# EvolBioInf/andi

Hardware: AMD Instinct MI355X
Metric: genome-pairs/sec (ordered pairs, n^2-n) over the N x N anchor-distance loop (higher is better)
Workload: dtype u8

## Files before the change

andi_amd/csrc/api.hip:

```cpp
#include <hip/hip_runtime.h>

#include <algorithm>
#include <atomic>
#include <chrono>
#include <cstdarg>
#include <cstdio>
#include <cstdlib>
#include <cstring>
#include <mutex>
#include <string>
#include <thread>
#include <sys/mman.h>
#include <vector>

#include "api_internal.h"
#include "andi_dev.h"
#include "andi_hip.h"
#include "bootstrap.h"
#include "dev_arena.h"
#include "esa_build.h"
#include "knobs.h"
#include "sa_device.h"
#include "scan.h"

// ... 620 lines not shown
	return 0;
}

int andi_hip_esa_build_index(andi_hip_ctx *ctx, andi_hip_esa *e) {
	if (!ctx || !e) return 1;
	HIP_TRY(ctx, hipSetDevice(ctx->device));
	Timed t(ctx, 0);
	const int ext = andi_index_single_ext(ctx->queries_hint, e->rec_valid);
	hipError_t err = andi_launch_index_build(build_args(e), ext, ctx->stream);
	t.stop();
	if (err == hipSuccess) err = hipEventRecord(ctx->built, ctx->stream);
	if (err != hipSuccess) return fail(ctx, "andi_hip_esa_build_index", err);
	e->index_built = true, e->deep_ext = (ext == 2 && !e->rec_valid) ? 0 : ext, ctx->builds_pending = true;
	return 0;
}

int andi_hip_esa_build_index_batch(andi_hip_ctx *ctx, andi_hip_esa *const *esas, size_t count) {
	if (!ctx || !esas || count == 0 || count > 65535) {
		if (ctx) ctx->err = "andi_hip_esa_build_index_batch: bad arguments";
		return 1;
	}
	HIP_TRY(ctx, hipSetDevice(ctx->device));
	if (ctx->ib_cap < count) {
		HIP_TRY(ctx, hipStreamSynchronize(ctx->stream));
		if (ctx->ib_dev) (void)andi_arena::dev_free(ctx->ib_dev);
		if (ctx->ib_host) host_pool::pinned_put(ctx->ib_host, ctx->ib_cap * sizeof(AndiIndexBatchItem));
		ctx->ib_dev = ctx->ib_host = nullptr, ctx->ib_cap = 0;
		const size_t cap = std::max<size_t>(count, 64);
		HIP_TRY(ctx, andi_arena::dev_malloc(&ctx->ib_dev, cap * sizeof(AndiIndexBatchItem)));
		HIP_TRY(ctx, host_pool::pinned_get(&ctx->ib_host, cap * sizeof(AndiIndexBatchItem)));
		if (!ctx->ib_done) HIP_TRY(ctx, hipEventCreateWithFlags(&ctx->ib_done, hipEventDisableTiming));
		ctx->ib_cap = cap;
	} else {
		HIP_TRY(ctx, hipEventSynchronize(ctx->ib_done));
	}
	auto *items = (AndiIndexBatchItem *)ctx->ib_host;
	int32_t max_n = 0;
	for (size_t k = 0; k < count; ++k) {
		andi_hip_esa *e = esas[k];
		if (!e) {
			ctx->err = "andi_hip_esa_build_index_batch: null subject";
			return 1;
		}
		items[k].S = e->S, items[k].SA = e->SA, items[k].deep = e->deep, items[k].N0 = e->N0, items[k].N1 = e->N1, items[k].P = e->P;
		items[k].flags = e->flags, items[k].n = e->n, items[k].deepK = e->deepK;
		items[k].rec = e->rec_valid ? e->rec : nullptr;
		items[k].rec2 = e->rec_valid ? e->rec2 : nullptr;
		items[k].single_ext = andi_index_single_ext(ctx->queries_hint, e->rec_valid);
		max_n = std::max(max_n, e->n);
	}
	Timed t(ctx, 0);
	hipError_t err = hipMemcpyAsync(ctx->ib_dev, ctx->ib_host, count * sizeof(AndiIndexBatchItem), hipMemcpyHostToDevice, ctx->stream);
	if (err == hipSuccess) err = hipEventRecord(ctx->ib_done, ctx->stream);
	if (err == hipSuccess) err = andi_launch_index_build_batch((const AndiIndexBatchItem *)ctx->ib_dev, (uint32_t)count, max_n, ctx->stream);
	t.stop();
	if (err == hipSuccess) err = hipEventRecord(ctx->built, ctx->stream);
	if (err != hipSuccess) return fail(ctx, "andi_hip_esa_build_index_batch", err);
	for (size_t k = 0; k < count; ++k) {
		const int ext = items[k].single_ext;
		esas[k]->index_built = true, esas[k]->deep_ext = (ext == 2 && !esas[k]->rec_valid) ? 0 : ext;
	}
	ctx->builds_pending = true;
	return 0;
}

int andi_hip_esa_flags(andi_hip_ctx *ctx, const andi_hip_esa *e, int32_t *out4) {
	if (!ctx || !e || !out4) return 1;
	HIP_TRY(ctx, hipStreamSynchronize(ctx->stream));
	memcpy(out4, e->h_flags, 4 * sizeof(int32_t));
	return 0;
}

int andi_hip_esa_download(andi_hip_ctx *ctx, const andi_hip_esa *e, int32_t *LCP, int32_t *CLD,
						  uint8_t *FVC, andi_hip_interval *cache) {
	if (!ctx || !e) return 1;
	if (!e->ref_built) {
		ctx->err = "andi_hip_esa_download: reference arrays not built (call andi_hip_esa_build)";
		return 1;
	}
	const size_t n = (size_t)e->n;
	HIP_TRY(ctx, hipStreamSynchronize(ctx->stream));
	if (LCP) HIP_TRY(ctx, hipMemcpy(LCP, e->LCP, (n + 1) * 4, hipMemcpyDeviceToHost));
	if (CLD) HIP_TRY(ctx, hipMemcpy(CLD, e->CLD, (n + 1) * 4, hipMemcpyDeviceToHost));
	if (FVC) HIP_TRY(ctx, hipMemcpy(FVC, e->FVC, n, hipMemcpyDeviceToHost));
	if (cache)
		HIP_TRY(ctx, hipMemcpy(cache, e->tab, ((size_t)16 << (2 * ANDI_CACHE_K)), hipMemcpyDeviceToHost));
	return 0;
}

int andi_hip_esa_download_index(andi_hip_ctx *ctx, const andi_hip_esa *e, uint32_t *table, int *K) {
	if (!ctx || !e) return 1;
	if (!e->index_built) {
		ctx->err = "andi_hip_esa_download_index: scan index not built (call andi_hip_esa_build_index)";
		return 1;
	}
	if (K) *K = e->deepK;
	HIP_TRY(ctx, hipStreamSynchronize(ctx->stream));
	if (table) HIP_TRY(ctx, hipMemcpy(table, e->deep, (size_t)8 << (2 * e->deepK), hipMemcpyDeviceToHost));
	return 0;
}

int andi_hip_esa_single_form(const andi_hip_esa *e) { return e && e->index_built ? e->deep_ext : 0; }

void andi_hip_esa_free(andi_hip_ctx *ctx, andi_hip_esa *e) {
	if (!e) return;
	if (ctx) (void)hipSetDevice(ctx->device);
	(void)hipDeviceSynchronize();
// ... 407 lines not shown
```

andi_amd/csrc/esa_build.h:

```cpp
#pragma once
#include <hip/hip_runtime.h>
#include <stdint.h>

#define ANDI_MIN_LEVELS 6

struct MinTree {
	const int32_t *lv[ANDI_MIN_LEVELS];
	int32_t cnt[ANDI_MIN_LEVELS];
	int levels;
};

struct EsaBuildArgs {
	const uint8_t *S;
	const int32_t *SA;
	int32_t *LCP;
	int32_t *CLD;
	uint8_t *FVC;
	int4 *tab;
	uint2 *deep;
	uint8_t *N0, *N1;
	uint32_t *P;
	int32_t *flags;
	const uint32_t *rec;
	const uint16_t *rec2;
	int32_t deepK;
	int32_t *min_scratch;
	int32_t n;
};

struct AndiIndexBatchItem {
	const uint8_t *S;
	const int32_t *SA;
	uint2 *deep;
	uint8_t *N0, *N1;
	uint32_t *P;
	int32_t *flags;
	const uint32_t *rec;
	const uint16_t *rec2;
	int32_t n, deepK;
	int32_t single_ext;
};

size_t andi_min_tree_entries(int32_t n);
int andi_index_single_ext(size_t queries, bool sorted_on_device);
hipError_t andi_launch_index_build_batch(const AndiIndexBatchItem *d_items, uint32_t count, int32_t max_n, hipStream_t st);
hipError_t andi_launch_pack_symbols_batch(const AndiIndexBatchItem *d_items, uint32_t count, size_t bytes, hipStream_t st);
hipError_t andi_launch_pack_planes_batch(const AndiIndexBatchItem *d_items, uint32_t count, size_t max_n, hipStream_t st);
hipError_t andi_launch_esa_build(const EsaBuildArgs &a, hipStream_t st);
hipError_t andi_launch_index_build(const EsaBuildArgs &a, int single_ext, hipStream_t st);
hipError_t andi_launch_rs_from_query(uint8_t *RS, const uint8_t *q, uint32_t len, hipStream_t st);
hipError_t andi_launch_gc_counts(const uint8_t *pool, const uint64_t *d_off, const uint32_t *d_len, uint32_t nq, uint32_t longest,
								 unsigned long long *d_counts, hipStream_t st);
hipError_t andi_launch_sep_counts(const uint8_t *pool, const uint64_t *d_off, const uint32_t *d_len, uint32_t nq, uint32_t longest,
								  uint32_t *d_counts, hipStream_t st);
```

andi_amd/csrc/esa_build.hip:

```cpp
#include "andi_dev.h"
#include "esa_build.h"
#include "scan.h"
#include "knobs.h"

#include <cstring>

#define CHECK_LAUNCH()                                                                             \
	do {                                                                                           \
		hipError_t e_ = hipGetLastError();                                                         \
		if (e_ != hipSuccess) return e_;                                                           \
	} while (0)

__global__ __launch_bounds__(256) void k_phi_scatter(const int32_t *__restrict__ SA,
													 int32_t *__restrict__ phi, int32_t n) {
	int32_t r = blockIdx.x * blockDim.x + threadIdx.x;
	if (r >= n) return;
	int32_t prev = r ? SA[r - 1] : -1;
	phi[SA[r]] = prev;
}

#define PLCP_CHUNK 32
__global__ __launch_bounds__(256) void k_plcp_chunks(const uint8_t *__restrict__ S,
													 int32_t *__restrict__ phi_plcp, int32_t n) {
	int64_t chunk = (int64_t)blockIdx.x * blockDim.x + threadIdx.x;
// ... 197 lines not shown
	}
	auto squeeze = [](uint32_t x) {
		x &= 0x33333333u;
		x = (x | (x >> 2)) & 0x0f0f0f0fu;
		x = (x | (x >> 4)) & 0x00ff00ffu;
		x = (x | (x >> 8)) & 0x0000ffffu;
		return x;
	};
	uint32_t y = __brev(squeeze((uint32_t)w) | (squeeze((uint32_t)(w >> 32)) << 16));
	y = ((y & 0x55555555u) << 1) | ((y >> 1) & 0x55555555u);
	return ((y >> (32 - 2 * K)) << 6) | (sep << 4) | v;
}

__device__ __forceinline__ uint32_t rec_lcp(uint32_t a, uint32_t b, int K) {
	uint32_t x = REC_CODE(a) ^ REC_CODE(b);
	uint32_t same = x ? (uint32_t)(__builtin_clz(x) - (32 - 2 * K)) >> 1 : (uint32_t)K;
	uint32_t va = REC_V(a), vb = REC_V(b);
	uint32_t m = va < vb ? va : vb;
	return same < m ? same : m;
}

__device__ __forceinline__ uint32_t rec_lcp_code(uint32_t code, uint32_t a, int K) {
	uint32_t x = code ^ REC_CODE(a);
	uint32_t same = x ? (uint32_t)(__builtin_clz(x) - (32 - 2 * K)) >> 1 : (uint32_t)K;
	uint32_t va = REC_V(a);
	return same < va ? same : va;
}

#ifndef PT_BLOCK
#define PT_BLOCK 256
#endif
#ifndef PT_GAPS
#define PT_GAPS 3
#endif
#define PT_TILE (PT_BLOCK * PT_GAPS)
#define PT_WORDS (PT_TILE / 64)
#define PT_RANKED 4096
__device__ __forceinline__ uint32_t wave_scan_incl(uint32_t v) {
	v += (uint32_t)__builtin_amdgcn_update_dpp(0, (int)v, 0x111, 0xf, 0xf, false);
	v += (uint32_t)__builtin_amdgcn_update_dpp(0, (int)v, 0x112, 0xf, 0xf, false);
	v += (uint32_t)__builtin_amdgcn_update_dpp(0, (int)v, 0x114, 0xf, 0xf, false);
	v += (uint32_t)__builtin_amdgcn_update_dpp(0, (int)v, 0x118, 0xf, 0xf, false);
	v += (uint32_t)__builtin_amdgcn_update_dpp(0, (int)v, 0x142, 0xa, 0xf, false);
	v += (uint32_t)__builtin_amdgcn_update_dpp(0, (int)v, 0x143, 0xc, 0xf, false);
	return v;
}

__device__ __forceinline__ uint32_t first_code(bool has, uint32_t L, int K) {
	const uint32_t v = REC_V(L), sh = 2 * ((uint32_t)K - v);
	const uint32_t c = ((REC_CODE(L) >> sh) << sh) + (v == (uint32_t)K ? 1u : 0u);
	return has ? c : 0u;
}

__device__ __forceinline__ void probe_table_block(const uint8_t *__restrict__ N0, const int32_t *__restrict__ SA,
												  const uint32_t *__restrict__ REC, const uint16_t *__restrict__ REC2, uint2 *__restrict__ deep,
												  int32_t *__restrict__ flags, int32_t n, int K, int single_ext, uint32_t block) {
	__shared__ uint32_t s_first[PT_TILE];
	__shared__ uint32_t s_absent[PT_TILE];
	__shared__ uint32_t s_h[PT_TILE + 2];
	__shared__ uint2 s_present[PT_TILE];
	__shared__ uint32_t s_rec[PT_TILE + 5];
	__shared__ uint64_t s_some[PT_WORDS];
	__shared__ uint32_t s_bits[PT_RANKED / 32];
	__shared__ uint32_t s_before[PT_RANKED / 32];
	__shared__ uint16_t s_owner[PT_TILE];

	const uint32_t r0 = block * PT_TILE;
	const uint32_t lane = threadIdx.x & 63u, wave = threadIdx.x >> 6;
	auto make_rec = [&](int32_t j) { return REC ? REC[j] : suffix_rec(N0, SA, j, K); };
	uint32_t mine2[PT_GAPS];
	{
		uint32_t mine[PT_GAPS];
#pragma unroll
		for (int u = 0; u < PT_GAPS; ++u) {
			const uint32_t g = r0 + threadIdx.x + u * PT_BLOCK;
			mine[u] = g < (uint32_t)n ? make_rec((int32_t)g) : 0u;
			mine2[u] = (single_ext == 2 && REC2 && g < (uint32_t)n) ? REC2[g] : 0u;
		}
#pragma unroll
		for (int u = 0; u < PT_GAPS; ++u) s_rec[threadIdx.x + u * PT_BLOCK + 2] = mine[u];
	}
	if (threadIdx.x < 2) s_rec[threadIdx.x] = r0 + threadIdx.x >= 2 ? make_rec((int32_t)(r0 + threadIdx.x - 2)) : 0u;
	if (threadIdx.x == 2) s_rec[PT_TILE + 2] = r0 + PT_TILE < (uint32_t)n ? make_rec((int32_t)(r0 + PT_TILE)) : 0u;
	if (threadIdx.x < PT_RANKED / 32) s_bits[threadIdx.x] = 0;
	__syncthreads();
	auto rec = [&](int32_t j) {
		const uint32_t k = (uint32_t)j - r0 + 2;
		return k < PT_TILE + 3 ? s_rec[k] : make_rec(j);
	};
	const uint32_t full = (uint32_t)K;
	if (threadIdx.x == 0) s_h[0] = r0 >= 2 ? rec_lcp(s_rec[0], s_rec[1], K) : 0u;
	if (threadIdx.x == 1) s_h[PT_TILE + 1] = r0 + PT_TILE < (uint32_t)n ? rec_lcp(s_rec[PT_TILE + 1], s_rec[PT_TILE + 2], K) : 0u;

	uint32_t counts[PT_GAPS], firsts[PT_GAPS];
#pragma unroll
	for (int u = 0; u < PT_GAPS; ++u) {
		const uint32_t i = threadIdx.x + u * PT_BLOCK;
		const uint32_t gid = r0 + i;
		const bool live = gid <= (uint32_t)n;
		const int32_t r = (int32_t)(live ? gid : 0);
		const bool hasL = live && r > 0, hasR = live && r < n;
		const uint32_t Lr = s_rec[i + 1], Rr = s_rec[i + 2], a1 = s_rec[i + 3], a2 = s_rec[i + 4], a3 = s_rec[i + 5];
		const uint32_t L = hasL ? Lr : 0u, R = hasR ? Rr : 0u;
		const uint32_t sa_r = hasR ? (uint32_t)SA[r] : 0u;
		const uint32_t h = (hasL && hasR) ? rec_lcp(L, R, K) : 0u;
		s_h[i + 1] = h;
		uint32_t absent = 0, first = 1u << (2 * K), owns_present = 0;
		uint2 present = make_uint2(0, 0);

		if (live) {
			if (hasR && REC_V(R) == full && !(hasL && L == R)) {
				const bool in_tile = i + 5 < PT_TILE + 3;
				const int32_t m = a1 != R ? 0 : (a2 != R ? 1 : (a3 != R ? 2 : 3));
				int32_t j = in_tile ? r + m : r;
				const bool more = !in_tile || m == 3;
				if (more) {
					while (j + 1 < n && j - r < 16 && rec(j + 1) == R) ++j;
					if (j - r == 16 && j + 1 < n && rec(j + 1) == R) {
						int32_t lo = j + 1, hi = n - 1;
						while (lo < hi) {
							const int32_t mid = lo + ((hi - lo + 1) >> 1);
							if (rec(mid) == R) lo = mid; else hi = mid - 1;
						}
						j = lo;
					}
				}
				if (j == r) {
					const uint32_t pos = sa_r, e0 = pos + full;
					if (single_ext == 2 && REC2) {
						const uint32_t w = mine2[u];
						present = make_uint2(pos, DEEP_SINGLE | ((w >> 8) << 2) | ((w & 0xffu) << 6));
					} else if (single_ext != 1) {
						present = make_uint2(pos, DEEP_SINGLE | (1u << 2) | (full << 8));
					} else {
						const uint64_t w = ld_u64_unaligned((g_u8p)N0 + (e0 >> 1)) >> (4 * (e0 & 1u));
						uint32_t nval = (uint32_t)__builtin_ctzll((w & 0x4444444444444444ull) | (1ull << 52)) >> 2;
						auto squeeze = [](uint32_t x) {
							x &= 0x33333333u;
							x = (x | (x >> 2)) & 0x0f0f0f0fu;
							x = (x | (x >> 4)) & 0x00ff00ffu;
							x = (x | (x >> 8)) & 0x0000ffffu;
							return x;
						};
						const uint32_t ext = (squeeze((uint32_t)w) | (squeeze((uint32_t)(w >> 32)) << 16)) & ((1u << (2 * nval)) - 1u);
						present = make_uint2(pos, DEEP_SINGLE | (nval << 2) | (ext << 6));
					}
				} else {
					const bool fits = (uint32_t)(j - r) < (1u << 24);
					present = make_uint2(fits ? (uint32_t)r : 0u, fits ? DEEP_MULTI | ((uint32_t)(j - r) << 8) : (uint32_t)DEEP_SEARCH);
				}
				owns_present = 1;
			}

			if (__builtin_amdgcn_ballot_w64(hasR && (REC_SEP(R) == 1 || REC_SEP(R) == 2)) != 0 && hasR) {
				uint32_t k = REC_V(R), sp = REC_SEP(R);
				if (k >= 1 && k <= 8 && k < full && (sp == 1 || sp == 2) && (!hasL || h < k)) {
					int32_t j = r;
					while (j + 1 < n) {
						uint32_t X = rec(j + 1);
						if (REC_V(X) == k && REC_SEP(X) == sp && rec_lcp(R, X, K) == k) ++j; else break;
					}
					if (j > r && (j + 1 == n || rec_lcp(R, rec(j + 1), K) < k)) flags[0] = 1;
				}
			}

			const int32_t lo = (int32_t)first_code(hasL, L, K);
			const uint32_t shR = 2 * (full - REC_V(R));
			const int32_t hi = hasR ? (int32_t)((REC_CODE(R) >> shR) << shR) - 1 : (int32_t)((1u << (2 * K)) - 1u);
			if (lo <= hi) absent = (uint32_t)(hi - lo + 1);
			first = (uint32_t)lo;
		}
		s_first[i] = first, s_absent[i] = absent, s_present[i] = present;
		counts[u] = absent + owns_present, firsts[u] = first;
		const uint64_t b = __ballot(counts[u] != 0);
		if (lane == 0) s_some[u * (PT_BLOCK / 64) + wave] = b;
	}

	__syncthreads();
	const uint32_t base = first_code(r0 > 0, s_rec[1], K);
	const uint32_t total = (r0 + PT_TILE <= (uint32_t)n ? first_code(true, s_rec[PT_TILE + 1], K) : (1u << (2 * K))) - base;
	uint32_t owners_before;
	{
		const uint32_t mine = lane < PT_WORDS ? (uint32_t)__builtin_popcountll(s_some[lane]) : 0u;
		owners_before = wave_scan_incl(mine) - mine;
	}
#pragma unroll
	for (int u = 0; u < PT_GAPS; ++u) {
		const uint32_t word = u * (PT_BLOCK / 64) + wave;
		const uint32_t before = (uint32_t)__builtin_amdgcn_readlane((int)owners_before, __builtin_amdgcn_readfirstlane((int)word));
		if (counts[u] == 0) continue;
		const uint32_t i = threadIdx.x + u * PT_BLOCK, off = firsts[u] - base;
		s_owner[before + (uint32_t)__builtin_popcountll(s_some[word] & ((1ull << lane) - 1ull))] = (uint16_t)i;
		if (off < PT_RANKED) atomicOr(&s_bits[off >> 5], 1u << (off & 31u));
	}
	__syncthreads();
	if (wave == 0) {
		uint32_t carry = 0;
		for (uint32_t w0 = 0; w0 < PT_RANKED / 32; w0 += 64) {
			const uint32_t mine = (uint32_t)__builtin_popcount(s_bits[w0 + lane]), incl = wave_scan_incl(mine);
			s_before[w0 + lane] = carry + incl - mine;
			carry += (uint32_t)__builtin_amdgcn_readlane((int)incl, 63);
		}
	}
	__syncthreads();

	auto write_entry = [&](uint32_t t, uint32_t a) {
		const uint32_t c = base + t;
		const bool is_present = c - s_first[a] >= s_absent[a];
		const uint2 pres = s_present[a];
		const uint32_t rr = r0 + a;
		const bool gL = rr > 0, gR = rr < (uint32_t)n;
		const uint32_t gl = s_rec[a + 1], gr = s_rec[a + 2], hll = s_h[a], hrr = s_h[a + 2];
		const uint32_t xL = rec_lcp_code(c, gl, K), xR = rec_lcp_code(c, gr, K);
		const uint32_t lL = gL ? xL : 0u, lR = gR ? xR : 0u;
		const bool left = lL > lR, right = lR > lL;
		const uint32_t l = left ? lL : lR;
		const uint32_t idx = left ? rr - 1 : (right ? rr : 0u);
		const bool alone = left ? (rr < 2 || hll < l) : (rr + 1 >= (uint32_t)n || hrr < l);
		const uint32_t uniq = ((left || right) && l != 0) ? (alone ? 1u : 0u) : (n == 1 ? 1u : 0u);
		const uint2 val = is_present ? pres : make_uint2(idx, DEEP_FINAL | (uniq << 2) | (l << 8));
		__builtin_nontemporal_store(((unsigned long long)val.y << 32) | val.x, (unsigned long long *)(deep + c));
	};
	const uint32_t ranked = total < PT_RANKED ? total : PT_RANKED;
	for (uint32_t t = threadIdx.x; t < ranked; t += PT_BLOCK) {
		const uint32_t word = t >> 5;
		write_entry(t, s_owner[s_before[word] + (uint32_t)__builtin_popcount(s_bits[word] & (0xffffffffu >> (31u - (t & 31u)))) - 1u]);
	}
	for (uint32_t t = PT_RANKED + threadIdx.x; t < total; t += PT_BLOCK) {
		const uint32_t c = base + t;
		uint32_t a = 0, b = PT_TILE;
		while (b - a > 1) {
			const uint32_t mid = (a + b) >> 1;
			if (s_first[mid] <= c) a = mid; else b = mid;
		}
		write_entry(t, a);
	}
}

__global__ __launch_bounds__(PT_BLOCK) void k_probe_table(const uint8_t *__restrict__ N0, const int32_t *__restrict__ SA,
														  const uint32_t *__restrict__ rec, const uint16_t *__restrict__ rec2, uint2 *__restrict__ deep,
														  int32_t *__restrict__ flags, int32_t n, int K, int single_ext) {
	probe_table_block(N0, SA, rec, rec2, deep, flags, n, K, single_ext, blockIdx.x);
}

__global__ __launch_bounds__(PT_BLOCK) void k_probe_table_batch(const AndiIndexBatchItem *__restrict__ items) {
	const AndiIndexBatchItem it = items[blockIdx.y];
	if ((uint64_t)blockIdx.x * PT_TILE > (uint64_t)it.n) return;
	probe_table_block(it.N0, it.SA, it.rec, it.rec2, it.deep, it.flags, it.n, it.deepK, it.single_ext, blockIdx.x);
}

size_t andi_min_tree_entries(int32_t n) {
	size_t total = 0;
	size_t cnt = (size_t)n + 1;
	while (cnt > 64) {
		cnt = (cnt + 63) / 64;
		total += cnt;
	}
	return total ? total : 1;
}

int andi_index_single_ext(size_t queries, bool sorted_on_device) {
	const int coop = andi_coop_enabled();
	if (coop == 0) return 0;
	if (sorted_on_device) return 2;
	return (coop > 0 || queries >= 256) ? 1 : 0;
}

hipError_t andi_launch_index_build(const EsaBuildArgs &a, int single_ext, hipStream_t st) {
	const int32_t n = a.n;
	hipError_t e;
	e = andi_launch_pack_symbols(a.S, (size_t)n + 1 + 64, a.N0, a.N1, a.flags + 1, st);
	if (e != hipSuccess) return e;
	if (a.P) e = andi_launch_pack_planes(a.N0, (size_t)n + 1 + 64, a.P, st);
	if (e != hipSuccess) return e;
	k_probe_table<<<(unsigned)(((int64_t)n + 1 + PT_TILE - 1) / PT_TILE), PT_BLOCK, 0, st>>>(a.N0, a.SA, a.rec, a.rec2, a.deep, a.flags, n,
																				  a.deepK, single_ext);
	CHECK_LAUNCH();
	return hipSuccess;
}

hipError_t andi_launch_index_build_batch(const AndiIndexBatchItem *d_items, uint32_t count, int32_t max_n, hipStream_t st) {
	if (count == 0) return hipSuccess;
	hipError_t e = andi_launch_pack_symbols_batch(d_items, count, (size_t)max_n + 1 + 64, st);
	if (e != hipSuccess) return e;
	e = andi_launch_pack_planes_batch(d_items, count, (size_t)max_n, st);
	if (e != hipSuccess) return e;
	const dim3 grid((unsigned)(((int64_t)max_n + 1 + PT_TILE - 1) / PT_TILE), count);
	k_probe_table_batch<<<grid, PT_BLOCK, 0, st>>>(d_items);
	CHECK_LAUNCH();
	return hipSuccess;
}

hipError_t andi_launch_esa_build(const EsaBuildArgs &a, hipStream_t st) {
	const int32_t n = a.n;
	const int B = 256;
	auto blocks = [&](int64_t items) { return (unsigned)((items + B - 1) / B); };

	int32_t *plcp = a.CLD;
	k_phi_scatter<<<blocks(n), B, 0, st>>>(a.SA, plcp, n);
	CHECK_LAUNCH();
	int64_t chunks = ((int64_t)n + PLCP_CHUNK - 1) / PLCP_CHUNK;
	k_plcp_chunks<<<blocks(chunks), B, 0, st>>>(a.S, plcp, n);
	CHECK_LAUNCH();
	k_lcp_fvc<<<blocks((int64_t)n + 1), B, 0, st>>>(a.S, a.SA, plcp, a.LCP, a.FVC, n);
	CHECK_LAUNCH();

	MinTree t;
	t.lv[0] = a.LCP;
	t.cnt[0] = n + 1;
	t.levels = 1;
	int32_t *next = a.min_scratch;
	while (t.cnt[t.levels - 1] > 64 && t.levels < ANDI_MIN_LEVELS) {
		int32_t in_cnt = t.cnt[t.levels - 1];
		int32_t out_cnt = (in_cnt + 63) / 64;
		k_min64<<<blocks(in_cnt), B, 0, st>>>(t.lv[t.levels - 1], in_cnt, next);
		CHECK_LAUNCH();
		t.lv[t.levels] = next;
		t.cnt[t.levels] = out_cnt;
		next += out_cnt;
		t.levels++;
	}
	hipError_t e = hipMemsetAsync(a.CLD, 0xff, ((size_t)n + 1) * sizeof(int32_t), st);
	if (e != hipSuccess) return e;
	k_child_table<<<blocks(n), B, 0, st>>>(t, a.CLD, n);
	CHECK_LAUNCH();

	EsaDev E;
	memset(&E, 0, sizeof E);
	E.S = a.S, E.SA = a.SA, E.LCP = a.LCP, E.CLD = a.CLD, E.FVC = a.FVC, E.tab = a.tab;
	E.flags = a.flags;
	E.n = n, E.mode = ANDI_MODE_REFERENCE;
	k_kmer_table<<<blocks(1 << (2 * ANDI_CACHE_K)), B, 0, st>>>(E, a.tab, a.flags);
	CHECK_LAUNCH();
	return hipSuccess;
}

__global__ __launch_bounds__(256) void k_rs_from_query(uint8_t *__restrict__ RS, const uint8_t *__restrict__ q, uint32_t len) {
	const uint64_t w = (uint64_t)blockIdx.x * 256 + threadIdx.x, o = 4 * w, n = 2 * (uint64_t)len + 1;
	if (o >= n) return;
	uint32_t word = 0;
#pragma unroll
// ... 90 lines not shown
```

andi_amd/csrc/scan_lane.hip:

```cpp
#include "lane_chain.h"
#include "knobs.h"

#include <algorithm>

namespace {

[[maybe_unused]] constexpr uint32_t EST_WAVES = 4;
constexpr uint32_t EST_WAVES_FEW = 8;
__global__ __launch_bounds__(64 * EST_WAVES_FEW) void k_pair_estimate(ScanArgs a, bool many) {
	__shared__ uint32_t s_shorts, s_runs;
	const uint32_t est_waves = many ? 1u : blockDim.x >> 6;
	const uint32_t pair = many ? blockIdx.x * (blockDim.x >> 6) + (threadIdx.x >> 6) : blockIdx.x, wave = many ? 0u : threadIdx.x >> 6;
	const uint32_t lane = threadIdx.x & 63u;
	if (pair >= a.nsub * a.nq) return;
	const uint32_t sub = pair / a.nq, qidx = pair % a.nq;
	const bool first = many ? lane == 0 : threadIdx.x == 0;
	if (a.self[sub] == (int64_t)qidx) {
		if (first) a.pair_class[pair] = 0, a.pair_waves[pair] = 0;
		return;
	}
	if (!many) {
		if (threadIdx.x == 0) s_shorts = 0, s_runs = 0;
		__syncthreads();
	}
// ... 860 lines not shown
	if ((bad & 0x80u) && foreign) *foreign = 1;
	N0[j] = make_uint2(w[0], w[1]);
	if (N1) {
		const uint32_t prev = j ? (lut[src[16 * j - 1]] & 7u) : 7u;
		N1[j] = make_uint2((w[0] << 4) | prev, (w[1] << 4) | (w[0] >> 28));
	}
}

__global__ __launch_bounds__(256) void k_pack_symbols(const uint8_t *__restrict__ src, int64_t pairs,
													  uint2 *__restrict__ N0, uint2 *__restrict__ N1,
													  int32_t *__restrict__ foreign) {
	pack_symbols_block(src, pairs, N0, N1, foreign);
}

__global__ __launch_bounds__(256) void k_unpack_symbols(const uint2 *__restrict__ N0, int64_t pairs, uint4 *__restrict__ dst) {
	const int64_t j = (int64_t)blockIdx.x * blockDim.x + threadIdx.x;
	if (j >= pairs) return;
	const uint2 v = N0[j];
	const uint64_t letters = 0x00233b2154474341ull;
	uint32_t out[4];
#pragma unroll
	for (int k = 0; k < 4; ++k) {
		const uint32_t w = (k < 2 ? v.x : v.y) >> (16 * (k & 1));
		uint32_t o = 0;
#pragma unroll
		for (int t = 0; t < 4; ++t) o |= (uint32_t)((letters >> (8 * ((w >> (4 * t)) & 7u))) & 0xffu) << (8 * t);
		out[k] = o;
	}
	dst[j] = make_uint4(out[0], out[1], out[2], out[3]);
}

__device__ __forceinline__ void planes_of(const uint4 v, uint32_t *out) {
	auto squeeze = [](uint32_t x) {
		x = (x >> 3) & 0x11111111u;
		x = (x | (x >> 3)) & 0x03030303u;
		x = (x | (x >> 6)) & 0x000f000fu;
		return (x | (x >> 12)) & 0xffu;
	};
#pragma unroll
	for (int b = 0; b < 3; ++b) {
		const int sh = 3 - b;
		out[b] = squeeze(v.x << sh) | (squeeze(v.y << sh) << 8) | (squeeze(v.z << sh) << 16) | (squeeze(v.w << sh) << 24);
	}
}

__global__ __launch_bounds__(256) void k_pack_planes(const uint4 *__restrict__ N0, int64_t blocks, uint32_t *__restrict__ planes) {
	const int64_t j = (int64_t)blockIdx.x * blockDim.x + threadIdx.x;
	if (j >= blocks) return;
	uint32_t o[3];
	planes_of(N0[j], o);
	planes[3 * j] = o[0], planes[3 * j + 1] = o[1], planes[3 * j + 2] = o[2];
}

__global__ __launch_bounds__(256) void k_pack_planes_batch(const AndiIndexBatchItem *__restrict__ items) {
	const AndiIndexBatchItem it = items[blockIdx.y];
	if (!it.P || !it.N0) return;
	const int64_t blocks = ((int64_t)it.n + 1 + 64 + 31) / 32, j = (int64_t)blockIdx.x * blockDim.x + threadIdx.x;
	if (j >= blocks) return;
	uint32_t o[3];
	planes_of(((const uint4 *)it.N0)[j], o);
	it.P[3 * j] = o[0], it.P[3 * j + 1] = o[1], it.P[3 * j + 2] = o[2];
}

__global__ __launch_bounds__(256) void k_pack_symbols_batch(const AndiIndexBatchItem *__restrict__ items) {
	const AndiIndexBatchItem it = items[blockIdx.y];
	pack_symbols_block(it.S, ((int64_t)it.n + 1 + 64 + 15) / 16, (uint2 *)it.N0, (uint2 *)it.N1, it.flags + 1);
}

}

#ifdef ANDI_QUAD_TU
hipError_t andi_launch_lane_quad_small(const ScanArgs &a0, uint32_t count, hipStream_t st) {
	if (count == 0) return hipSuccess;
	ScanArgs a = a0;
	a.quad_listed = 1;
	if (a.exact_equal)
		k_lane_quad<true><<<count, BLOCK, 0, st>>>(a);
	else
		k_lane_quad<false><<<count, BLOCK, 0, st>>>(a);
	return hipGetLastError();
}
#else

hipError_t andi_launch_pack_symbols_batch(const AndiIndexBatchItem *d_items, uint32_t count, size_t bytes, hipStream_t st) {
	const int64_t pairs = (int64_t)((bytes + 15) / 16);
	if (pairs == 0 || count == 0) return hipSuccess;
	k_pack_symbols_batch<<<dim3((unsigned)((pairs + 255) / 256), count), 256, 0, st>>>(d_items);
	CHECK_LAUNCH();
	return hipSuccess;
}

hipError_t andi_launch_unpack_symbols(const uint8_t *N0, size_t bytes, uint8_t *dst, hipStream_t st) {
	const int64_t pairs = (int64_t)(bytes / 16);
	if (pairs == 0) return hipSuccess;
	k_unpack_symbols<<<(unsigned)((pairs + 255) / 256), 256, 0, st>>>((const uint2 *)N0, pairs, (uint4 *)dst);
	CHECK_LAUNCH();
	return hipSuccess;
}

hipError_t andi_launch_pack_planes(const uint8_t *N0, size_t symbols, uint32_t *planes, hipStream_t st) {
	const int64_t blocks = (int64_t)((symbols + 31) / 32);
	if (blocks == 0) return hipSuccess;
	k_pack_planes<<<(unsigned)((blocks + 255) / 256), 256, 0, st>>>((const uint4 *)N0, blocks, planes);
	CHECK_LAUNCH();
	return hipSuccess;
}

hipError_t andi_launch_pack_planes_batch(const AndiIndexBatchItem *d_items, uint32_t count, size_t max_n, hipStream_t st) {
	const int64_t blocks = (int64_t)((max_n + 1 + 64 + 31) / 32);
	if (blocks == 0 || count == 0) return hipSuccess;
	k_pack_planes_batch<<<dim3((unsigned)((blocks + 255) / 256), count), 256, 0, st>>>(d_items);
	CHECK_LAUNCH();
	return hipSuccess;
}

hipError_t andi_launch_pack_symbols(const uint8_t *src, size_t bytes, uint8_t *N0, uint8_t *N1,
									int32_t *foreign, hipStream_t st) {
	const int64_t pairs = (int64_t)((bytes + 15) / 16);
	if (pairs == 0) return hipSuccess;
	k_pack_symbols<<<(unsigned)((pairs + 255) / 256), 256, 0, st>>>(src, pairs, (uint2 *)N0, (uint2 *)N1, foreign);
	CHECK_LAUNCH();
	return hipSuccess;
}

template <bool EXACT>
static hipError_t lane_cold(const ScanArgs &a, dim3 grid, hipStream_t st) {
	const bool blocks4 = andi_knob(KNOB_QUAD_UNLISTED) != nullptr;
	const bool quads = a.adaptive && a.quad_min_match != 0xffffffffu;
	const bool side = quads && a.side_stream && !andi_knob(KNOB_NO_SIDE_STREAM);
	const bool counted = side && a.h_quad_waves && !blocks4 && !andi_knob(KNOB_QUAD_BLOCKS4);
	if (quads) {
		(void)hipMemsetAsync(a.first_pub, 0xff, (size_t)64 * a.max_waves * sizeof(unsigned long long), st);
		if (side) {
			(void)hipEventRecord(a.side_fork, st);
			(void)hipStreamWaitEvent(a.side_stream, a.side_fork, 0);
		}
		if (!counted) {
			ScanArgs b = a;
			b.quad_listed = blocks4 ? 0 : 1;
			k_lane_quad<EXACT><<<grid, BLOCK, 0, side ? a.side_stream : st>>>(b);
			if (side) (void)hipEventRecord(a.side_join, a.side_stream);
		}
	}
	if (a.adaptive) k_lane_cold<EXACT, true><<<grid, BLOCK, 0, st>>>(a);
	else k_lane_cold<EXACT, false><<<grid, BLOCK, 0, st>>>(a);
	hipError_t e = hipSuccess;
	if (counted) {
		(void)hipMemcpyAsync(a.h_quad_waves, a.restitch_count + ANDI_QUAD_WAVES, sizeof(uint32_t), hipMemcpyDeviceToHost, a.side_stream);
		e = hipStreamSynchronize(a.side_stream);
		if (e == hipSuccess) e = andi_launch_lane_quad_small(a, *a.h_quad_waves, a.side_stream);
		(void)hipEventRecord(a.side_join, a.side_stream);
	}
	if (side) (void)hipStreamWaitEvent(st, a.side_join, 0);
	return e != hipSuccess ? e : hipGetLastError();
}

static hipError_t pair_offsets(const ScanArgs &a, hipStream_t st) {
	const uint32_t P = a.nsub * a.nq;
	const unsigned nb = (P + 1023) / 1024;
	k_pair_block_sums<<<nb, 1024, 0, st>>>(a);
	CHECK_LAUNCH();
	k_pair_block_offsets<<<1, 1024, 0, st>>>(a);
	CHECK_LAUNCH();
	k_pair_offsets<<<nb, 1024, 0, st>>>(a);
// ... 157 lines not shown
```

Measured before the change: 138,100.

## Fuse symbol and plane packing, specialize probe table with hot template path

After: 145,800, median of 6. 5.6% higher.

```diff
diff --git a/andi_amd/csrc/api.hip b/andi_amd/csrc/api.hip
--- a/andi_amd/csrc/api.hip
+++ b/andi_amd/csrc/api.hip
@@ -696,7 +696,7 @@
 	Timed t(ctx, 0);
 	hipError_t err = hipMemcpyAsync(ctx->ib_dev, ctx->ib_host, count * sizeof(AndiIndexBatchItem), hipMemcpyHostToDevice, ctx->stream);
 	if (err == hipSuccess) err = hipEventRecord(ctx->ib_done, ctx->stream);
-	if (err == hipSuccess) err = andi_launch_index_build_batch((const AndiIndexBatchItem *)ctx->ib_dev, (uint32_t)count, max_n, ctx->stream);
+	if (err == hipSuccess) err = andi_launch_index_build_batch(items, (const AndiIndexBatchItem *)ctx->ib_dev, (uint32_t)count, max_n, ctx->stream);
 	t.stop();
 	if (err == hipSuccess) err = hipEventRecord(ctx->built, ctx->stream);
 	if (err != hipSuccess) return fail(ctx, "andi_hip_esa_build_index_batch", err);
diff --git a/andi_amd/csrc/esa_build.h b/andi_amd/csrc/esa_build.h
--- a/andi_amd/csrc/esa_build.h
+++ b/andi_amd/csrc/esa_build.h
@@ -43,9 +43,9 @@
 
 size_t andi_min_tree_entries(int32_t n);
 int andi_index_single_ext(size_t queries, bool sorted_on_device);
-hipError_t andi_launch_index_build_batch(const AndiIndexBatchItem *d_items, uint32_t count, int32_t max_n, hipStream_t st);
-hipError_t andi_launch_pack_symbols_batch(const AndiIndexBatchItem *d_items, uint32_t count, size_t bytes, hipStream_t st);
-hipError_t andi_launch_pack_planes_batch(const AndiIndexBatchItem *d_items, uint32_t count, size_t max_n, hipStream_t st);
+hipError_t andi_launch_index_build_batch(const AndiIndexBatchItem *h_items, const AndiIndexBatchItem *d_items, uint32_t count, int32_t max_n, hipStream_t st);
+hipError_t andi_launch_pack_forms_batch(const AndiIndexBatchItem *d_items, uint32_t count, size_t bytes, hipStream_t st);
+hipError_t andi_launch_pack_forms(const uint8_t *src, size_t bytes, uint8_t *N0, uint8_t *N1, uint32_t *P, int32_t *foreign, hipStream_t st);
 hipError_t andi_launch_esa_build(const EsaBuildArgs &a, hipStream_t st);
 hipError_t andi_launch_index_build(const EsaBuildArgs &a, int single_ext, hipStream_t st);
 hipError_t andi_launch_rs_from_query(uint8_t *RS, const uint8_t *q, uint32_t len, hipStream_t st);
diff --git a/andi_amd/csrc/esa_build.hip b/andi_amd/csrc/esa_build.hip
--- a/andi_amd/csrc/esa_build.hip
+++ b/andi_amd/csrc/esa_build.hip
@@ -273,14 +273,13 @@
 	return has ? c : 0u;
 }
 
+template <bool HOT>
 __device__ __forceinline__ void probe_table_block(const uint8_t *__restrict__ N0, const int32_t *__restrict__ SA,
 												  const uint32_t *__restrict__ REC, const uint16_t *__restrict__ REC2, uint2 *__restrict__ deep,
 												  int32_t *__restrict__ flags, int32_t n, int K, int single_ext, uint32_t block) {
-	__shared__ uint32_t s_first[PT_TILE];
-	__shared__ uint32_t s_absent[PT_TILE];
 	__shared__ uint32_t s_h[PT_TILE + 2];
 	__shared__ uint2 s_present[PT_TILE];
-	__shared__ uint32_t s_rec[PT_TILE + 5];
+	__shared__ uint32_t s_rec[PT_TILE + 3];
 	__shared__ uint64_t s_some[PT_WORDS];
 	__shared__ uint32_t s_bits[PT_RANKED / 32];
 	__shared__ uint32_t s_before[PT_RANKED / 32];
@@ -288,7 +287,8 @@
 
 	const uint32_t r0 = block * PT_TILE;
 	const uint32_t lane = threadIdx.x & 63u, wave = threadIdx.x >> 6;
-	auto make_rec = [&](int32_t j) { return REC ? REC[j] : suffix_rec(N0, SA, j, K); };
+	auto make_rec = [&](int32_t j) { return HOT ? REC[j] : (REC ? REC[j] : suffix_rec(N0, SA, j, K)); };
+	const bool short_ext = HOT || (single_ext == 2 && REC2);
 	uint32_t mine2[PT_GAPS];
 	{
 		uint32_t mine[PT_GAPS];
@@ -296,7 +296,7 @@
 		for (int u = 0; u < PT_GAPS; ++u) {
 			const uint32_t g = r0 + threadIdx.x + u * PT_BLOCK;
 			mine[u] = g < (uint32_t)n ? make_rec((int32_t)g) : 0u;
-			mine2[u] = (single_ext == 2 && REC2 && g < (uint32_t)n) ? REC2[g] : 0u;
+			mine2[u] = (short_ext && g < (uint32_t)n) ? REC2[g] : 0u;
 		}
 #pragma unroll
 		for (int u = 0; u < PT_GAPS; ++u) s_rec[threadIdx.x + u * PT_BLOCK + 2] = mine[u];
@@ -312,8 +312,10 @@
 	const uint32_t full = (uint32_t)K;
 	if (threadIdx.x == 0) s_h[0] = r0 >= 2 ? rec_lcp(s_rec[0], s_rec[1], K) : 0u;
 	if (threadIdx.x == 1) s_h[PT_TILE + 1] = r0 + PT_TILE < (uint32_t)n ? rec_lcp(s_rec[PT_TILE + 1], s_rec[PT_TILE + 2], K) : 0u;
-
-	uint32_t counts[PT_GAPS], firsts[PT_GAPS];
+	const uint32_t base = first_code(r0 > 0, s_rec[1], K);
+	const uint32_t total = (r0 + PT_TILE <= (uint32_t)n ? first_code(true, s_rec[PT_TILE + 1], K) : (1u << (2 * K))) - base;
+
+	uint32_t counts[PT_GAPS];
 #pragma unroll
 	for (int u = 0; u < PT_GAPS; ++u) {
 		const uint32_t i = threadIdx.x + u * PT_BLOCK;
@@ -321,23 +323,31 @@
 		const bool live = gid <= (uint32_t)n;
 		const int32_t r = (int32_t)(live ? gid : 0);
 		const bool hasL = live && r > 0, hasR = live && r < n;
-		const uint32_t Lr = s_rec[i + 1], Rr = s_rec[i + 2], a1 = s_rec[i + 3], a2 = s_rec[i + 4], a3 = s_rec[i + 5];
+		const uint32_t Lr = s_rec[i + 1], Rr = s_rec[i + 2];
+		const bool ahead = i + 64 <= PT_TILE;
+		const uint32_t La = s_rec[ahead ? i + 65 : 0], Ra = s_rec[ahead ? i + 66 : 0];
 		const uint32_t L = hasL ? Lr : 0u, R = hasR ? Rr : 0u;
 		const uint32_t sa_r = hasR ? (uint32_t)SA[r] : 0u;
 		const uint32_t h = (hasL && hasR) ? rec_lcp(L, R, K) : 0u;
 		s_h[i + 1] = h;
+		const uint64_t ends0 = __ballot(Lr != Rr), ends1 = __ballot(ahead && La != Ra);
 		uint32_t absent = 0, first = 1u << (2 * K), owns_present = 0;
 		uint2 present = make_uint2(0, 0);
 
 		if (live) {
 			if (hasR && REC_V(R) == full && !(hasL && L == R)) {
-				const bool in_tile = i + 5 < PT_TILE + 3;
-				const int32_t m = a1 != R ? 0 : (a2 != R ? 1 : (a3 != R ? 2 : 3));
-				int32_t j = in_tile ? r + m : r;
-				const bool more = !in_tile || m == 3;
-				if (more) {
-					while (j + 1 < n && j - r < 16 && rec(j + 1) == R) ++j;
-					if (j - r == 16 && j + 1 < n && rec(j + 1) == R) {
+				const uint64_t mine0 = (ends0 >> 1) >> lane;
+				int32_t j;
+				if (mine0 != 0) {
+					j = r + (int32_t)__builtin_ctzll(mine0);
+				} else if (ends1 != 0) {
+					j = r + (int32_t)(63u - lane) + (int32_t)__builtin_ctzll(ends1);
+				} else {
+					const uint32_t known = i - lane + 127u < PT_TILE ? i - lane + 127u : PT_TILE;
+					j = (int32_t)(r0 + known);
+					const int32_t j0 = j;
+					while (j + 1 < n && j - j0 < 16 && rec(j + 1) == R) ++j;
+					if (j - j0 == 16 && j + 1 < n && rec(j + 1) == R) {
 						int32_t lo = j + 1, hi = n - 1;
 						while (lo < hi) {
 							const int32_t mid = lo + ((hi - lo + 1) >> 1);
@@ -348,7 +358,7 @@
 				}
 				if (j == r) {
 					const uint32_t pos = sa_r, e0 = pos + full;
-					if (single_ext == 2 && REC2) {
+					if (short_ext) {
 						const uint32_t w = mine2[u];
 						present = make_uint2(pos, DEEP_SINGLE | ((w >> 8) << 2) | ((w & 0xffu) << 6));
 					} else if (single_ext != 1) {
@@ -391,15 +401,14 @@
 			if (lo <= hi) absent = (uint32_t)(hi - lo + 1);
 			first = (uint32_t)lo;
 		}
-		s_first[i] = first, s_absent[i] = absent, s_present[i] = present;
-		counts[u] = absent + owns_present, firsts[u] = first;
+		s_present[i] = present;
+		counts[u] = absent + owns_present;
 		const uint64_t b = __ballot(counts[u] != 0);
 		if (lane == 0) s_some[u * (PT_BLOCK / 64) + wave] = b;
-	}
-
+		const uint32_t off = first - base;
+		if (counts[u] != 0 && off < PT_RANKED) atomicOr(&s_bits[off >> 5], 1u << (off & 31u));
+	}
 	__syncthreads();
-	const uint32_t base = first_code(r0 > 0, s_rec[1], K);
-	const uint32_t total = (r0 + PT_TILE <= (uint32_t)n ? first_code(true, s_rec[PT_TILE + 1], K) : (1u << (2 * K))) - base;
 	uint32_t owners_before;
 	{
 		const uint32_t mine = lane < PT_WORDS ? (uint32_t)__builtin_popcountll(s_some[lane]) : 0u;
@@ -410,11 +419,8 @@
 		const uint32_t word = u * (PT_BLOCK / 64) + wave;
 		const uint32_t before = (uint32_t)__builtin_amdgcn_readlane((int)owners_before, __builtin_amdgcn_readfirstlane((int)word));
 		if (counts[u] == 0) continue;
-		const uint32_t i = threadIdx.x + u * PT_BLOCK, off = firsts[u] - base;
-		s_owner[before + (uint32_t)__builtin_popcountll(s_some[word] & ((1ull << lane) - 1ull))] = (uint16_t)i;
-		if (off < PT_RANKED) atomicOr(&s_bits[off >> 5], 1u << (off & 31u));
-	}
-	__syncthreads();
+		s_owner[before + (uint32_t)__builtin_popcountll(s_some[word] & ((1ull << lane) - 1ull))] = (uint16_t)(threadIdx.x + u * PT_BLOCK);
+	}
 	if (wave == 0) {
 		uint32_t carry = 0;
 		for (uint32_t w0 = 0; w0 < PT_RANKED / 32; w0 += 64) {
@@ -427,11 +433,11 @@
 
 	auto write_entry = [&](uint32_t t, uint32_t a) {
 		const uint32_t c = base + t;
-		const bool is_present = c - s_first[a] >= s_absent[a];
 		const uint2 pres = s_present[a];
 		const uint32_t rr = r0 + a;
 		const bool gL = rr > 0, gR = rr < (uint32_t)n;
 		const uint32_t gl = s_rec[a + 1], gr = s_rec[a + 2], hll = s_h[a], hrr = s_h[a + 2];
+		const bool is_present = REC_V(gr) == full && c == REC_CODE(gr);
 		const uint32_t xL = rec_lcp_code(c, gl, K), xR = rec_lcp_code(c, gr, K);
 		const uint32_t lL = gL ? xL : 0u, lR = gR ? xR : 0u;
 		const bool left = lL > lR, right = lR > lL;
@@ -447,28 +453,33 @@
 		const uint32_t word = t >> 5;
 		write_entry(t, s_owner[s_before[word] + (uint32_t)__builtin_popcount(s_bits[word] & (0xffffffffu >> (31u - (t & 31u)))) - 1u]);
 	}
+	auto gap_first = [&](uint32_t i) { return r0 + i <= (uint32_t)n ? first_code(r0 + i > 0, s_rec[i + 1], K) : 1u << (2 * K); };
 	for (uint32_t t = PT_RANKED + threadIdx.x; t < total; t += PT_BLOCK) {
 		const uint32_t c = base + t;
 		uint32_t a = 0, b = PT_TILE;
 		while (b - a > 1) {
 			const uint32_t mid = (a + b) >> 1;
-			if (s_first[mid] <= c) a = mid; else b = mid;
+			if (gap_first(mid) <= c) a = mid; else b = mid;
 		}
 		write_entry(t, a);
 	}
 }
 
+template <bool HOT>
 __global__ __launch_bounds__(PT_BLOCK) void k_probe_table(const uint8_t *__restrict__ N0, const int32_t *__restrict__ SA,
 														  const uint32_t *__restrict__ rec, const uint16_t *__restrict__ rec2, uint2 *__restrict__ deep,
 														  int32_t *__restrict__ flags, int32_t n, int K, int single_ext) {
-	probe_table_block(N0, SA, rec, rec2, deep, flags, n, K, single_ext, blockIdx.x);
-}
-
+	probe_table_block<HOT>(N0, SA, rec, rec2, deep, flags, n, K, single_ext, blockIdx.x);
+}
+
+template <bool HOT>
 __global__ __launch_bounds__(PT_BLOCK) void k_probe_table_batch(const AndiIndexBatchItem *__restrict__ items) {
 	const AndiIndexBatchItem it = items[blockIdx.y];
 	if ((uint64_t)blockIdx.x * PT_TILE > (uint64_t)it.n) return;
-	probe_table_block(it.N0, it.SA, it.rec, it.rec2, it.deep, it.flags, it.n, it.deepK, it.single_ext, blockIdx.x);
-}
+	probe_table_block<HOT>(it.N0, it.SA, it.rec, it.rec2, it.deep, it.flags, it.n, it.deepK, it.single_ext, blockIdx.x);
+}
+
+static bool probe_table_hot(const uint32_t *rec, const uint16_t *rec2, int single_ext) { return rec && rec2 && single_ext == 2; }
 
 size_t andi_min_tree_entries(int32_t n) {
 	size_t total = 0;
@@ -490,24 +501,28 @@
 hipError_t andi_launch_index_build(const EsaBuildArgs &a, int single_ext, hipStream_t st) {
 	const int32_t n = a.n;
 	hipError_t e;
-	e = andi_launch_pack_symbols(a.S, (size_t)n + 1 + 64, a.N0, a.N1, a.flags + 1, st);
+	e = andi_launch_pack_forms(a.S, (size_t)n + 1 + 64, a.N0, a.N1, a.P, a.flags + 1, st);
 	if (e != hipSuccess) return e;
-	if (a.P) e = andi_launch_pack_planes(a.N0, (size_t)n + 1 + 64, a.P, st);
-	if (e != hipSuccess) return e;
-	k_probe_table<<<(unsigned)(((int64_t)n + 1 + PT_TILE - 1) / PT_TILE), PT_BLOCK, 0, st>>>(a.N0, a.SA, a.rec, a.rec2, a.deep, a.flags, n,
-																				  a.deepK, single_ext);
+	const unsigned grid = (unsigned)(((int64_t)n + 1 + PT_TILE - 1) / PT_TILE);
+	if (probe_table_hot(a.rec, a.rec2, single_ext))
+		k_probe_table<true><<<grid, PT_BLOCK, 0, st>>>(a.N0, a.SA, a.rec, a.rec2, a.deep, a.flags, n, a.deepK, single_ext);
+	else
+		k_probe_table<false><<<grid, PT_BLOCK, 0, st>>>(a.N0, a.SA, a.rec, a.rec2, a.deep, a.flags, n, a.deepK, single_ext);
 	CHECK_LAUNCH();
 	return hipSuccess;
 }
 
-hipError_t andi_launch_index_build_batch(const AndiIndexBatchItem *d_items, uint32_t count, int32_t max_n, hipStream_t st) {
+hipError_t andi_launch_index_build_batch(const AndiIndexBatchItem *h_items, const AndiIndexBatchItem *d_items, uint32_t count, int32_t max_n, hipStream_t st) {
 	if (count == 0) return hipSuccess;
-	hipError_t e = andi_launch_pack_symbols_batch(d_items, count, (size_t)max_n + 1 + 64, st);
-	if (e != hipSuccess) return e;
-	e = andi_launch_pack_planes_batch(d_items, count, (size_t)max_n, st);
+	hipError_t e = andi_launch_pack_forms_batch(d_items, count, (size_t)max_n + 1 + 64, st);
 	if (e != hipSuccess) return e;
 	const dim3 grid((unsigned)(((int64_t)max_n + 1 + PT_TILE - 1) / PT_TILE), count);
-	k_probe_table_batch<<<grid, PT_BLOCK, 0, st>>>(d_items);
+	bool hot = true;
+	for (uint32_t k = 0; k < count; ++k) hot = hot && probe_table_hot(h_items[k].rec, h_items[k].rec2, h_items[k].single_ext);
+	if (hot)
+		k_probe_table_batch<true><<<grid, PT_BLOCK, 0, st>>>(d_items);
+	else
+		k_probe_table_batch<false><<<grid, PT_BLOCK, 0, st>>>(d_items);
 	CHECK_LAUNCH();
 	return hipSuccess;
 }
diff --git a/andi_amd/csrc/scan_lane.hip b/andi_amd/csrc/scan_lane.hip
--- a/andi_amd/csrc/scan_lane.hip
+++ b/andi_amd/csrc/scan_lane.hip
@@ -936,19 +936,52 @@
 	planes[3 * j] = o[0], planes[3 * j + 1] = o[1], planes[3 * j + 2] = o[2];
 }
 
-__global__ __launch_bounds__(256) void k_pack_planes_batch(const AndiIndexBatchItem *__restrict__ items) {
+__device__ __forceinline__ void pack_forms_block(const uint8_t *__restrict__ src, int64_t pairs, uint2 *__restrict__ N0,
+												 uint2 *__restrict__ N1, uint32_t *__restrict__ P, int32_t *__restrict__ foreign) {
+	__shared__ uint8_t lut[256];
+	lut[threadIdx.x] = (uint8_t)(symbol_of((uint8_t)threadIdx.x) | (in_alphabet((uint8_t)threadIdx.x) ? 0u : 0x80u));
+	__syncthreads();
+	const int64_t j = (int64_t)blockIdx.x * blockDim.x + threadIdx.x;
+	if (2 * j >= pairs) return;
+	const bool two = 2 * j + 1 < pairs;
+	const uint4 v0 = ld_u128_unaligned((g_u8p)src + 32 * j);
+	const uint4 v1 = two ? ld_u128_unaligned((g_u8p)src + 32 * j + 16) : make_uint4(0, 0, 0, 0);
+	const uint32_t prev = j ? (lut[src[32 * j - 1]] & 7u) : 7u;
+	const uint32_t in[8] = {v0.x, v0.y, v0.z, v0.w, v1.x, v1.y, v1.z, v1.w};
+	uint32_t w[4] = {0, 0, 0, 0}, bad = 0;
+#pragma unroll
+	for (int k = 0; k < 32; ++k) {
+		const uint32_t e = lut[(in[k >> 2] >> (8 * (k & 3))) & 0xffu];
+		w[k >> 3] |= (e & 7u) << (4 * (k & 7));
+		bad |= e;
+	}
+	if ((bad & 0x80u) && foreign) *foreign = 1;
+	if (two) {
+		((uint4 *)N0)[j] = make_uint4(w[0], w[1], w[2], w[3]);
+		if (N1) ((uint4 *)N1)[j] = make_uint4((w[0] << 4) | prev, (w[1] << 4) | (w[0] >> 28), (w[2] << 4) | (w[1] >> 28), (w[3] << 4) | (w[2] >> 28));
+	} else {
+		N0[2 * j] = make_uint2(w[0], w[1]);
+		if (N1) N1[2 * j] = make_uint2((w[0] << 4) | prev, (w[1] << 4) | (w[0] >> 28));
+		if (P) {
+			const uint2 behind = N0[2 * j + 1];
+			w[2] = behind.x, w[3] = behind.y;
+		}
+	}
+	if (P) {
+		uint32_t o[3];
+		planes_of(make_uint4(w[0], w[1], w[2], w[3]), o);
+		P[3 * j] = o[0], P[3 * j + 1] = o[1], P[3 * j + 2] = o[2];
+	}
+}
+
+__global__ __launch_bounds__(256) void k_pack_forms(const uint8_t *__restrict__ src, int64_t pairs, uint2 *__restrict__ N0,
+													uint2 *__restrict__ N1, uint32_t *__restrict__ P, int32_t *__restrict__ foreign) {
+	pack_forms_block(src, pairs, N0, N1, P, foreign);
+}
+
+__global__ __launch_bounds__(256) void k_pack_forms_batch(const AndiIndexBatchItem *__restrict__ items) {
 	const AndiIndexBatchItem it = items[blockIdx.y];
-	if (!it.P || !it.N0) return;
-	const int64_t blocks = ((int64_t)it.n + 1 + 64 + 31) / 32, j = (int64_t)blockIdx.x * blockDim.x + threadIdx.x;
-	if (j >= blocks) return;
-	uint32_t o[3];
-	planes_of(((const uint4 *)it.N0)[j], o);
-	it.P[3 * j] = o[0], it.P[3 * j + 1] = o[1], it.P[3 * j + 2] = o[2];
-}
-
-__global__ __launch_bounds__(256) void k_pack_symbols_batch(const AndiIndexBatchItem *__restrict__ items) {
-	const AndiIndexBatchItem it = items[blockIdx.y];
-	pack_symbols_block(it.S, ((int64_t)it.n + 1 + 64 + 15) / 16, (uint2 *)it.N0, (uint2 *)it.N1, it.flags + 1);
+	pack_forms_block(it.S, ((int64_t)it.n + 1 + 64 + 15) / 16, (uint2 *)it.N0, (uint2 *)it.N1, it.P, it.flags + 1);
 }
 
 }
@@ -966,10 +999,18 @@
 }
 #else
 
-hipError_t andi_launch_pack_symbols_batch(const AndiIndexBatchItem *d_items, uint32_t count, size_t bytes, hipStream_t st) {
-	const int64_t pairs = (int64_t)((bytes + 15) / 16);
-	if (pairs == 0 || count == 0) return hipSuccess;
-	k_pack_symbols_batch<<<dim3((unsigned)((pairs + 255) / 256), count), 256, 0, st>>>(d_items);
+hipError_t andi_launch_pack_forms_batch(const AndiIndexBatchItem *d_items, uint32_t count, size_t bytes, hipStream_t st) {
+	const int64_t blocks = (int64_t)((bytes + 31) / 32);
+	if (blocks == 0 || count == 0) return hipSuccess;
+	k_pack_forms_batch<<<dim3((unsigned)((blocks + 255) / 256), count), 256, 0, st>>>(d_items);
+	CHECK_LAUNCH();
+	return hipSuccess;
+}
+
+hipError_t andi_launch_pack_forms(const uint8_t *src, size_t bytes, uint8_t *N0, uint8_t *N1, uint32_t *P, int32_t *foreign, hipStream_t st) {
+	const int64_t pairs = (int64_t)((bytes + 15) / 16), blocks = (pairs + 1) / 2;
+	if (pairs == 0) return hipSuccess;
+	k_pack_forms<<<(unsigned)((blocks + 255) / 256), 256, 0, st>>>(src, pairs, (uint2 *)N0, (uint2 *)N1, P, foreign);
 	CHECK_LAUNCH();
 	return hipSuccess;
 }
@@ -986,14 +1027,6 @@
 	const int64_t blocks = (int64_t)((symbols + 31) / 32);
 	if (blocks == 0) return hipSuccess;
 	k_pack_planes<<<(unsigned)((blocks + 255) / 256), 256, 0, st>>>((const uint4 *)N0, blocks, planes);
-	CHECK_LAUNCH();
-	return hipSuccess;
-}
-
-hipError_t andi_launch_pack_planes_batch(const AndiIndexBatchItem *d_items, uint32_t count, size_t max_n, hipStream_t st) {
-	const int64_t blocks = (int64_t)((max_n + 1 + 64 + 31) / 32);
-	if (blocks == 0 || count == 0) return hipSuccess;
-	k_pack_planes_batch<<<dim3((unsigned)((blocks + 255) / 256), count), 256, 0, st>>>(d_items);
 	CHECK_LAUNCH();
 	return hipSuccess;
 }
```

## Pack per-gap probe descriptors into compacted owner-ranked shared array

Applied to the files above, without the earlier changes.

Result: faster. 138,000 before, 142,400 after, median of 6 (+3.2%).

```diff
diff --git a/andi_amd/csrc/esa_build.hip b/andi_amd/csrc/esa_build.hip
--- a/andi_amd/csrc/esa_build.hip
+++ b/andi_amd/csrc/esa_build.hip
@@ -273,18 +273,26 @@
 	return has ? c : 0u;
 }
 
+__device__ __forceinline__ uint32_t pt_side(uint32_t rec, uint32_t sh) {
+	return (REC_CODE(rec) << sh) | (1u << (sh - 1u)) | REC_V(rec);
+}
+__device__ __forceinline__ uint32_t pt_side_lcp(uint32_t cs, uint32_t side) {
+	const uint32_t same = (uint32_t)__builtin_clz(cs ^ side) >> 1, v = side & 15u;
+	return same < v ? same : v;
+}
+
 __device__ __forceinline__ void probe_table_block(const uint8_t *__restrict__ N0, const int32_t *__restrict__ SA,
 												  const uint32_t *__restrict__ REC, const uint16_t *__restrict__ REC2, uint2 *__restrict__ deep,
 												  int32_t *__restrict__ flags, int32_t n, int K, int single_ext, uint32_t block) {
-	__shared__ uint32_t s_first[PT_TILE];
-	__shared__ uint32_t s_absent[PT_TILE];
-	__shared__ uint32_t s_h[PT_TILE + 2];
-	__shared__ uint2 s_present[PT_TILE];
-	__shared__ uint32_t s_rec[PT_TILE + 5];
+	__shared__ uint2 s_pool[PT_TILE + 4];
+	uint32_t *const s_rec = (uint32_t *)s_pool;
+	uint32_t *const s_h = s_rec + PT_TILE + 5;
+	uint2 *const s_pres = s_pool;
+	__shared__ uint4 s_desc[PT_TILE];
 	__shared__ uint64_t s_some[PT_WORDS];
 	__shared__ uint32_t s_bits[PT_RANKED / 32];
 	__shared__ uint32_t s_before[PT_RANKED / 32];
-	__shared__ uint16_t s_owner[PT_TILE];
+	static_assert(PT_TILE <= 1024 && sizeof(uint2) * (PT_TILE + 4) >= sizeof(uint32_t) * (2 * PT_TILE + 7), "descriptor fields, pool size");
 
 	const uint32_t r0 = block * PT_TILE;
 	const uint32_t lane = threadIdx.x & 63u, wave = threadIdx.x >> 6;
@@ -313,7 +321,9 @@
 	if (threadIdx.x == 0) s_h[0] = r0 >= 2 ? rec_lcp(s_rec[0], s_rec[1], K) : 0u;
 	if (threadIdx.x == 1) s_h[PT_TILE + 1] = r0 + PT_TILE < (uint32_t)n ? rec_lcp(s_rec[PT_TILE + 1], s_rec[PT_TILE + 2], K) : 0u;
 
-	uint32_t counts[PT_GAPS], firsts[PT_GAPS];
+	uint32_t firsts[PT_GAPS], ends[PT_GAPS];
+	uint2 pres[PT_GAPS];
+	bool owner[PT_GAPS];
 #pragma unroll
 	for (int u = 0; u < PT_GAPS; ++u) {
 		const uint32_t i = threadIdx.x + u * PT_BLOCK;
@@ -391,33 +401,44 @@
 			if (lo <= hi) absent = (uint32_t)(hi - lo + 1);
 			first = (uint32_t)lo;
 		}
-		s_first[i] = first, s_absent[i] = absent, s_present[i] = present;
-		counts[u] = absent + owns_present, firsts[u] = first;
-		const uint64_t b = __ballot(counts[u] != 0);
+		firsts[u] = first, ends[u] = (first + absent) | (owns_present << 31), pres[u] = present;
+		owner[u] = (absent | owns_present) != 0;
+		const uint64_t b = __ballot(owner[u]);
 		if (lane == 0) s_some[u * (PT_BLOCK / 64) + wave] = b;
 	}
 
 	__syncthreads();
 	const uint32_t base = first_code(r0 > 0, s_rec[1], K);
 	const uint32_t total = (r0 + PT_TILE <= (uint32_t)n ? first_code(true, s_rec[PT_TILE + 1], K) : (1u << (2 * K))) - base;
-	uint32_t owners_before;
+	uint32_t owners_before, owners;
 	{
 		const uint32_t mine = lane < PT_WORDS ? (uint32_t)__builtin_popcountll(s_some[lane]) : 0u;
-		owners_before = wave_scan_incl(mine) - mine;
-	}
+		const uint32_t incl = wave_scan_incl(mine);
+		owners_before = incl - mine;
+		owners = (uint32_t)__builtin_amdgcn_readlane((int)incl, PT_WORDS - 1);
+	}
+	const uint32_t shK = 32u - 2u * (uint32_t)K;
+	uint4 desc[PT_GAPS];
+#pragma unroll
+	for (int u = 0; u < PT_GAPS; ++u) {
+		const uint32_t i = threadIdx.x + u * PT_BLOCK;
+		desc[u] = make_uint4(ends[u] | (s_h[i] << 27), pt_side(s_rec[i + 1], shK), pt_side(s_rec[i + 2], shK), i | (s_h[i + 2] << 10));
+	}
+	__syncthreads();
 #pragma unroll
 	for (int u = 0; u < PT_GAPS; ++u) {
 		const uint32_t word = u * (PT_BLOCK / 64) + wave;
 		const uint32_t before = (uint32_t)__builtin_amdgcn_readlane((int)owners_before, __builtin_amdgcn_readfirstlane((int)word));
-		if (counts[u] == 0) continue;
-		const uint32_t i = threadIdx.x + u * PT_BLOCK, off = firsts[u] - base;
-		s_owner[before + (uint32_t)__builtin_popcountll(s_some[word] & ((1ull << lane) - 1ull))] = (uint16_t)i;
+		if (!owner[u]) continue;
+		const uint32_t rank = before + (uint32_t)__builtin_popcountll(s_some[word] & ((1ull << lane) - 1ull)), off = firsts[u] - base;
+		s_desc[rank] = desc[u], s_pres[rank] = pres[u];
 		if (off < PT_RANKED) atomicOr(&s_bits[off >> 5], 1u << (off & 31u));
 	}
 	__syncthreads();
+	const uint32_t ranked = total < PT_RANKED ? total : PT_RANKED;
 	if (wave == 0) {
 		uint32_t carry = 0;
-		for (uint32_t w0 = 0; w0 < PT_RANKED / 32; w0 += 64) {
+		for (uint32_t w0 = 0; w0 < (ranked + 31u) / 32u; w0 += 64) {
 			const uint32_t mine = (uint32_t)__builtin_popcount(s_bits[w0 + lane]), incl = wave_scan_incl(mine);
 			s_before[w0 + lane] = carry + incl - mine;
 			carry += (uint32_t)__builtin_amdgcn_readlane((int)incl, 63);
@@ -425,34 +446,33 @@
 	}
 	__syncthreads();
 
-	auto write_entry = [&](uint32_t t, uint32_t a) {
+	const uint32_t lone = n == 1 ? 1u : 0u;
+	auto write_entry = [&](uint32_t t, uint32_t j) {
 		const uint32_t c = base + t;
-		const bool is_present = c - s_first[a] >= s_absent[a];
-		const uint2 pres = s_present[a];
-		const uint32_t rr = r0 + a;
-		const bool gL = rr > 0, gR = rr < (uint32_t)n;
-		const uint32_t gl = s_rec[a + 1], gr = s_rec[a + 2], hll = s_h[a], hrr = s_h[a + 2];
-		const uint32_t xL = rec_lcp_code(c, gl, K), xR = rec_lcp_code(c, gr, K);
-		const uint32_t lL = gL ? xL : 0u, lR = gR ? xR : 0u;
+		const uint4 d = s_desc[j];
+		const uint2 pres = s_pres[j];
+		const bool is_present = c >= (d.x & 0x7ffffffu);
+		const uint32_t rr = r0 + (d.w & 1023u);
+		const uint32_t cs = c << shK;
+		const uint32_t lL = pt_side_lcp(cs, d.y), lR = pt_side_lcp(cs, d.z);
 		const bool left = lL > lR, right = lR > lL;
 		const uint32_t l = left ? lL : lR;
 		const uint32_t idx = left ? rr - 1 : (right ? rr : 0u);
-		const bool alone = left ? (rr < 2 || hll < l) : (rr + 1 >= (uint32_t)n || hrr < l);
-		const uint32_t uniq = ((left || right) && l != 0) ? (alone ? 1u : 0u) : (n == 1 ? 1u : 0u);
+		const uint32_t hn = left ? (d.x >> 27) & 15u : (d.w >> 10) & 15u;
+		const uint32_t uniq = (left || right) ? (hn < l ? 1u : 0u) : lone;
 		const uint2 val = is_present ? pres : make_uint2(idx, DEEP_FINAL | (uniq << 2) | (l << 8));
 		__builtin_nontemporal_store(((unsigned long long)val.y << 32) | val.x, (unsigned long long *)(deep + c));
 	};
-	const uint32_t ranked = total < PT_RANKED ? total : PT_RANKED;
 	for (uint32_t t = threadIdx.x; t < ranked; t += PT_BLOCK) {
 		const uint32_t word = t >> 5;
-		write_entry(t, s_owner[s_before[word] + (uint32_t)__builtin_popcount(s_bits[word] & (0xffffffffu >> (31u - (t & 31u)))) - 1u]);
+		write_entry(t, s_before[word] + (uint32_t)__builtin_popcount(s_bits[word] & (0xffffffffu >> (31u - (t & 31u)))) - 1u);
 	}
 	for (uint32_t t = PT_RANKED + threadIdx.x; t < total; t += PT_BLOCK) {
 		const uint32_t c = base + t;
-		uint32_t a = 0, b = PT_TILE;
-		while (b - a > 1) {
-			const uint32_t mid = (a + b) >> 1;
-			if (s_first[mid] <= c) a = mid; else b = mid;
+		uint32_t a = 0, b = owners - 1;
+		while (a < b) {
+			const uint32_t mid = (a + b) >> 1, x = s_desc[mid].x;
+			if ((x & 0x7ffffffu) + (x >> 31) > c) b = mid; else a = mid + 1;
 		}
 		write_entry(t, a);
 	}
```
